# Rouslan/NTracer

Measured on AMD Instinct MI355X. Metric: Mrays/s (primary+shadow), 6-D hypercube @1920x1080, higher is better.
Workload: dtype f32

## Files before the change

### ntracer_amd/csrc/nt_box.hpp

```cpp
#pragma once
#include <type_traits>
#include "nt_pixel.hpp"

namespace {

__device__ __forceinline__ bool box_may_hit(int n, const float *dots, float sx, float sy, float sq) {
    const float osq = dots[0];
    const float ov = fmaf(-dots[2], sy, fmaf(dots[1], sx, dots[3]));
    const float rad2 = (float)n * (1.0f + NT_FUZZ) * (1.0f + NT_FUZZ) * 1.001f;
#ifdef NT_EXP_SKIP_SLABS
    return false;
#else
    return !((osq - rad2) * sq > ov * ov * 1.0001f);
#endif
}

__device__ __forceinline__ void box_background(float in, float &r, float &g, float &b) {
    if (in > 0.0f) { r = in; g = in; b = in; }
    else { r = 0.0f; g = -in; b = -in; }
}

template <int N>
__device__ __forceinline__ void box_color(const float (&o)[N], const float (&dir)[N], bool maybe, float &r, float &g, float &b) {
    bool done = false;
// ... 51 lines not shown

#ifndef NT_BOX_INLINE_MAX_N
#define NT_BOX_INLINE_MAX_N 8
#endif
#ifndef NT_BOX_SETS_MAX_N
#define NT_BOX_SETS_MAX_N NT_BOX_INLINE_MAX_N
#endif
#ifndef NT_BOX_MARGIN
#define NT_BOX_MARGIN 1e-5f
#endif
template <int N>
__device__ __forceinline__ void box_classify(const float (&o)[N], const float (&v)[N], float m, bool maybe, bool &hit, bool &unclear,
                                             float &x, float (&near)[N], float &tn, float &vK) {
    float tn2 = -INFINITY;
    tn = -INFINITY;
    vK = 0.0f;
    float tnp = -INFINITY, tfp = INFINITY;
    const float m1p = 1.0f + m;
#pragma unroll
    for (int j = 0; j < N; ++j) {
        const float inv = __builtin_amdgcn_rcpf(v[j]);
        const float c0 = -o[j] * inv;
        const float nr = c0 - fabsf(inv);
        near[j] = nr;
        tnp = fmaxf(tnp, fmaf(-fabsf(inv), m1p, c0));
        tfp = fminf(tfp, fmaf(fabsf(inv), m1p, c0));
        const bool later = nr > tn;
        tn2 = __builtin_amdgcn_fmed3f(tn, tn2, nr);
        vK = later ? v[j] : vK;
        tn = fmaxf(tn, nr);
    }
    const bool miss = tnp > tfp || tfp < 0.0f;
    const float c = 1.0f - m;
    float sum = 0.0f;
#pragma unroll
    for (int j = 0; j < N; ++j) sum = sum + fmaxf(fabsf(fmaf(v[j], tn, o[j])), c);
    const bool inside = sum - (float)N * c <= 1.5f * m;
    const bool sole = (tn - tn2) * fabsf(vK) > m;
    const bool front = tn > 1e-3f && tn < 1e30f;
    hit = maybe && !miss && inside && sole && front;
    unclear = maybe && !miss && !hit;
#ifdef NT_EXP_NOUNCLEAR
    unclear = false;
#endif
    x = hit ? vK : v[0];
}

__device__ __forceinline__ float nt_vmax(float a, float b) { float r; asm("v_max_f32 %0, %1, %2" : "=v"(r) : "v"(a), "v"(b)); return r; }
__device__ __forceinline__ float nt_vmin(float a, float b) { float r; asm("v_min_f32 %0, %1, %2" : "=v"(r) : "v"(a), "v"(b)); return r; }
__device__ __forceinline__ float nt_vmax3(float a, float b, float c) { float r; asm("v_max3_f32 %0, %1, %2, %3" : "=v"(r) : "v"(a), "v"(b), "v"(c)); return r; }
__device__ __forceinline__ float nt_vmin3(float a, float b, float c) { float r; asm("v_min3_f32 %0, %1, %2, %3" : "=v"(r) : "v"(a), "v"(b), "v"(c)); return r; }
__device__ __forceinline__ float nt_vmed3(float a, float b, float c) { float r; asm("v_med3_f32 %0, %1, %2, %3" : "=v"(r) : "v"(a), "v"(b), "v"(c)); return r; }
__device__ __forceinline__ float nt_vmax_abs(float a, float b) { float r; asm("v_max_f32 %0, |%1|, %2" : "=v"(r) : "v"(a), "v"(b)); return r; }

#ifndef NT_BOX_CLASSIFY_SETS_MIN_N
#define NT_BOX_CLASSIFY_SETS_MIN_N 6
#endif
#ifndef NT_BOX_CLASSIFY_SETS_MAX_N
#define NT_BOX_CLASSIFY_SETS_MAX_N 7
#endif
template <int N>
__device__ __forceinline__ void box_classify_sets(const float (&o)[N], const float (&v)[N], float m, uint32_t sets, bool &hit, bool &unclear,
                                                  float &x) {
    float tn = -INFINITY, tn2 = -INFINITY, vK = 0.0f;
    float tnp = -INFINITY, tfp = INFINITY;
    const float m1p = 1.0f + m;
#pragma unroll
    for (int j = 0; j < N; ++j) {
        if (((sets >> (10 + j)) & 1u) != 0u) {
            const float inv = __builtin_amdgcn_rcpf(v[j]);
            const float c0 = -o[j] * inv;
            tfp = nt_vmin(tfp, fmaf(fabsf(inv), m1p, c0));
            if (((sets >> j) & 1u) != 0u) {
                const float nr = c0 - fabsf(inv);
                tnp = nt_vmax(tnp, fmaf(-fabsf(inv), m1p, c0));
                const bool later = nr > tn;
                tn2 = nt_vmed3(tn, tn2, nr);
                vK = later ? v[j] : vK;
                tn = nt_vmax(tn, nr);
            }
        }
    }
    const bool miss = tnp > tfp || tfp < 0.0f;
    const float c = 1.0f - m;
    float sum = 0.0f;
#ifndef NT_EXP_SETS_MASKS
    asm volatile("" : "+s"(sets));
#endif
#pragma unroll
    for (int j = 0; j < N; ++j) {
        if (((sets >> (10 + j)) & 1u) != 0u) {
            asm volatile("" : "+v"(sum));
            sum = sum + nt_vmax_abs(fmaf(v[j], tn, o[j]), c);
        }
    }
    const bool inside = sum - (float)__builtin_popcount((sets >> 10) & 0x3ffu) * c <= 1.5f * m;
    const bool sole = (tn - tn2) * fabsf(vK) > m;
    const bool front = tn > 1e-3f && tn < 1e30f;
    hit = !miss && inside && sole && front;
    unclear = !miss && !hit;
    x = hit ? vK : v[0];
}

template <int N>
__device__ __forceinline__ void box_entries(const float (&o)[N], const float (&v)[N], float (&near)[N], float &tn, float &vK) {
    tn = -INFINITY;
// ... 56 lines not shown
    }
}

typedef __attribute__((address_space(1))) uint8_t *nt_gptr;
__device__ __forceinline__ nt_gptr uniform_ptr(uint8_t *p) {
    const unsigned long long v = reinterpret_cast<unsigned long long>(p);
    const uint32_t lo = (uint32_t)__builtin_amdgcn_readfirstlane((int)(uint32_t)v), hi = (uint32_t)__builtin_amdgcn_readfirstlane((int)(uint32_t)(v >> 32));
    return (nt_gptr)(((unsigned long long)hi << 32) | lo);
}
#define NT_G32(p) (*(__attribute__((address_space(1))) uint32_t *)(p))

template <typename P>
__device__ __forceinline__ void emit_f32x3_at(const NtTarget &tg, P p, float r, float gb) {
    r = r > 0.0f ? r : 0.0f;
    r = r < 1.0f ? r : 1.0f;
    gb = gb > 0.0f ? gb : 0.0f;
    gb = gb < 1.0f ? gb : 1.0f;
    uint32_t vr = __float_as_uint(r), vgb = __float_as_uint(gb);
    uint3 w;
    if (tg.plain_f32[0] == 0 && tg.plain_f32[1] == 1 && tg.plain_f32[2] == 2 && !tg.reversed) {
        w.x = bswap32(vr);
        w.y = bswap32(vgb);
        w.z = w.y;
    } else {
        if (!tg.reversed) { vr = bswap32(vr); vgb = bswap32(vgb); }
        w.x = tg.plain_f32[tg.reversed ? 2 : 0] == 0 ? vr : vgb;
        w.y = tg.plain_f32[1] == 0 ? vr : vgb;
        w.z = tg.plain_f32[tg.reversed ? 0 : 2] == 0 ? vr : vgb;
    }
    if constexpr (std::is_same<P, nt_gptr>::value) {
        typedef uint32_t u32x3 __attribute__((ext_vector_type(3)));
        u32x3 v;
        v.x = w.x; v.y = w.y; v.z = w.z;
        *(__attribute__((address_space(1))) u32x3 *)(p) = v;
    } else {
        *reinterpret_cast<uint3 *>(p) = w;
    }
}
__device__ __forceinline__ void emit_f32x3(const NtTarget &tg, long long offset, float r, float gb) { emit_f32x3_at(tg, tg.dest + offset, r, gb); }

__device__ __forceinline__ float sqrt_in_range(float x) {
    const float s = __builtin_amdgcn_sqrtf(x);
    const float s_dn = __uint_as_float(__float_as_uint(s) - 1u), s_up = __uint_as_float(__float_as_uint(s) + 1u);
    const float vp = fmaf(-s_dn, s, x), vs = fmaf(-s_up, s, x);
    float r = vp <= 0.0f ? s_dn : s;
    r = vs > 0.0f ? s_up : r;
    return r;
}
__device__ __forceinline__ float sqrt_wave(float x) {
    if (__builtin_amdgcn_ballot_w64(!(x >= 0x1p-96f && x < 0x1p96f)) == 0ull) return sqrt_in_range(x);
    return sqrtf(x);
}

template <int N, bool PLAIN, bool DEFER = false, bool REDO = false, bool F32 = false>
__device__ __forceinline__ bool box_pixel(const NtTarget &tg, const PixelRef &pr, const float (&org)[N], float (&dir)[N], float sq,
                                          const float (&dots)[4], float sx, float sy, float margin, bool rowhit = true, int face = -1,
                                          uint32_t sets = 0u, bool noclass = false) {
    constexpr bool INL = (F32 || PLAIN) && !REDO && !DEFER;
    const bool redo = REDO || (INL && noclass);
    const bool maybe = redo || (rowhit && (DEFER || INL || box_may_hit(N, dots, sx, sy, sq)));
    float r, g, b;
    bool hit = false, unclear = false;
    float x = dir[0];
#ifndef NT_EXP_NOCLASSIFY
    float near[N], tn = 0.0f, vK = 0.0f;
    constexpr bool CSETS = INL && N >= NT_BOX_CLASSIFY_SETS_MIN_N && N <= NT_BOX_CLASSIFY_SETS_MAX_N;
    auto exact_on_sets = [&]() {
        const float len = sqrt_wave(sq);
        float d[N];
#pragma unroll
        for (int j = 0; j < N; ++j) {
            d[j] = 0.0f;
            if ((sets >> (10 + j)) & 1u) d[j] = dir[j] / len;
        }
        bool done = false;
        x = dir[0];
#pragma unroll
        for (int i = 0; i < N; ++i) {
            if (((sets >> i) & 1u) != 0u && __builtin_amdgcn_ballot_w64(!done) != 0ull) {
                const float di = d[i];
                const float dist = ((di < 0.0f ? 1.0f : -1.0f) - org[i]) / di;
                bool ok = !done && di != 0.0f && dist > 0.0f;
#pragma unroll
                for (int j = 0; j < N; ++j) {
                    if (j != i && ((sets >> (10 + j)) & 1u) != 0u) {
                        const float p = d[j] * dist + org[j];
                        ok = ok && !(fabsf(p) > (1.0f + NT_FUZZ));
                    }
                }
                if (ok) {
                    done = true;
                    if (!(dist >= FLT_MAX)) { hit = true; x = dir[i]; }
                }
            }
        }
    };
    if constexpr (CSETS) {
        const bool have_sets = face < 0 && (sets & 0x80000000u) != 0u;
        bool on_sets = have_sets && redo;
        bool sorted = face >= 0;
        if (face >= 0) {
            hit = true;
#pragma unroll
            for (int j = 1; j < N; ++j) x = face == j ? dir[j] : x;
        } else if (have_sets && !redo && __builtin_amdgcn_ballot_w64(maybe) != 0ull) {
            box_classify_sets<N>(org, dir, margin, sets, hit, unclear, x);
            on_sets = __builtin_amdgcn_ballot_w64(unclear) != 0ull;
            unclear = false;
            sorted = true;
        }
        if (on_sets) {
            hit = false;
            exact_on_sets();
        } else if (sorted) {
        } else if (redo) {
            box_entries<N>(org, dir, near, tn, vK);
            unclear = true;
        } else if (__builtin_amdgcn_ballot_w64(maybe) != 0ull) {
            box_classify<N>(org, dir, margin, maybe, hit, unclear, x, near, tn, vK);
        }
    } else {
        if (face >= 0) {
            hit = true;
#pragma unroll
            for (int j = 1; j < N; ++j) x = face == j ? dir[j] : x;
        } else if ((REDO || INL) && redo && (sets & 0x80000000u) != 0u) {
            exact_on_sets();
        } else if (redo) {
            box_entries<N>(org, dir, near, tn, vK);
            unclear = true;
        } else if (__builtin_amdgcn_ballot_w64(maybe) != 0ull) {
            box_classify<N>(org, dir, margin, maybe, hit, unclear, x, near, tn, vK);
        }
    }
    if (DEFER) {
        if (__builtin_amdgcn_ballot_w64(unclear) != 0ull) return false;
    } else {
        const bool hard = unclear && !(tn > 1e-3f && tn < 1e30f);
        if (__builtin_amdgcn_ballot_w64(unclear) != 0ull && __builtin_amdgcn_ballot_w64(hard) == 0ull) {
            box_resolve<N>(org, dir, sqrt_wave(sq), margin, near, tn, vK, unclear, hit, x);
            unclear = false;
        }
    }
#else
    unclear = maybe;
#endif
    if (__builtin_amdgcn_ballot_w64(unclear) == 0ull) {
        if (PLAIN || (plain_rgb(tg) && tg.plain_bits <= 10u)) {
            const float maxv = (float)tg.plain_maxval;
            const float t = (fabsf(x) * __builtin_amdgcn_rsqf(sq)) * maxv;
            const float tgb = hit ? t * 0.5f : t;
            const bool clear_gb = fabsf(__builtin_amdgcn_fractf(tgb) - 0.5f) > fmaf(tgb, 0x1p-20f, 0x1p-20f);
            const bool clear_r = fabsf(__builtin_amdgcn_fractf(t) - 0.5f) > fmaf(t, 0x1p-20f, 0x1p-20f);
            if (__builtin_amdgcn_ballot_w64(!(clear_gb && (clear_r || !hit))) == 0ull) {
                if (tg.plain_sel != 0u) {
                    const uint32_t q8gb = __float_as_uint(tgb + 8388608.0f), q8r = __float_as_uint(t + 8388608.0f);
                    *reinterpret_cast<uint32_t *>(tg.dest + pr.offset) = __builtin_amdgcn_perm((hit || x > 0.0f) ? q8r : 0u, q8gb, tg.plain_sel);
                    return true;
                }
                uint32_t qgb = (uint32_t)(tgb + 0.5f), qr = (uint32_t)(t + 0.5f);
                qgb = qgb < tg.plain_maxval ? qgb : tg.plain_maxval;
                qr = qr < tg.plain_maxval ? qr : tg.plain_maxval;
                emit_plain(tg, pr, (hit || x > 0.0f) ? qr : 0u, qgb);
                return true;
            }
        }
        const float in = x / sqrtf(sq);
        if (hit) {
            const float shade = fabsf(in);
            r = shade * 1.0f;
            g = shade * 0.5f;
            b = shade * 0.5f;
        } else {
            box_background(in, r, g, b);
        }
    } else if (!DEFER) {
        const float len = sqrtf(sq);
#pragma unroll
        for (int j = 0; j < N; ++j) dir[j] = dir[j] / len;
// ... 87 lines not shown
template <int N, int SPLIT>
__global__ __launch_bounds__(256) void box_redo_kernel(NtCameraFixed cam, NtTarget tg) {
    const int tid = (int)threadIdx.x;
    const int wv = __builtin_amdgcn_readfirstlane(tid >> 6);
    static_assert(SPLIT == 1 || SPLIT == 2 || SPLIT == 4, "waves per redo word");
    const int row = (int)blockIdx.y * (4 / SPLIT) + wv / SPLIT;
    if (row >= tg.row_count) return;
    uint32_t *word = tg.redo + ((size_t)blockIdx.z * tg.row_count + row) * tg.redo_words + blockIdx.x;
    const uint32_t mine = (SPLIT == 1 ? 0xffffffffu : SPLIT == 2 ? 0x55555555u : 0x11111111u) << (wv % SPLIT);
    uint32_t todo = *word & mine;
    if (todo == 0u) return;
    if ((tid & 63) == 0) {
        if (SPLIT > 1) atomicAnd(word, ~mine);
        else *word = 0u;
    }
    float org[N], right[N], up[N], fwd[N], dir[N];
    load_camera<N>(cam, org, right, up, fwd);
    float margin = fabsf(org[0]);
#pragma unroll
    for (int j = 1; j < N; ++j) margin = fmaxf(margin, fabsf(org[j]));
    margin = NT_BOX_MARGIN * (1.0f + margin);
    float dots[4];
    if (cam.buf) {
        const float *dp = cam.dots + (size_t)blockIdx.z * 4;
        dots[0] = dp[0]; dots[1] = dp[1]; dots[2] = dp[2]; dots[3] = dp[3];
    } else {
        dots[0] = cam.odots[0]; dots[1] = cam.odots[1]; dots[2] = cam.odots[2]; dots[3] = cam.odots[3];
    }
    const int orow = tg.row_begin + row;
    const int y = nt_image_row(tg, orow);
    if (y >= tg.height) return;
    const float sy = tg.fovI * ((float)y - tg.half_h);
    while (todo != 0u) {
        const int bit = __builtin_ctz(todo);
        todo &= todo - 1u;
        int x = ((int)blockIdx.x * 32 + bit) * 64 + (tid & 63);
        x = x < tg.width ? x : tg.width - 1;
        PixelRef pr;
        pr.x = x;
        pr.y = y;
        pr.offset = (long long)blockIdx.z * tg.frame_stride + (long long)(tg.compact ? orow : y) * tg.pitch + (long long)x * tg.bpp;
        pr.hit_index = 0;
        pr.valid = true;
        const float sx = tg.fovI * ((float)x - tg.half_w);
#pragma unroll
        for (int j = 0; j < N; ++j) dir[j] = (fwd[j] + right[j] * sx) - up[j] * sy;
        float sq = dir[0] * dir[0];
#pragma unroll
        for (int j = 1; j < N; ++j) sq = sq + dir[j] * dir[j];
        box_pixel<N, true, false, true>(tg, pr, org, dir, sq, dots, sx, sy, margin);
    }
}

template <int N, bool SETS = false>
__device__ __forceinline__ unsigned long long box_stretch_code2(const float (&org)[N], const float (&right)[N], const float (&up)[N],
                                                                const float (&fwd)[N], const NtTarget &tg, int y, int col) {
    uint32_t sets_value = 0u;
    uint32_t *const sets = SETS ? &sets_value : nullptr;
    uint32_t code = 0u;
    float omax = fabsf(org[0]);
#pragma unroll
    for (int j = 1; j < N; ++j) omax = fmaxf(omax, fabsf(org[j]));
    const float m = NT_BOX_MARGIN * (1.0f + omax);
    const float h = 1.0f + 2.0f * m + 1e-3f;
    const float sxc = tg.fovI * (((float)(col * 64) + 31.5f) - tg.half_w);
    const float sy = tg.fovI * ((float)y - tg.half_h);
    const float spread = 32.0f * tg.fovI;
    float tlo = 0.0f, thi = INFINITY;
    float vc[N], g[N];
    float tn = -INFINITY, tn2 = -INFINITY, vK = 0.0f, gK = 0.0f, oK = 0.0f;
    int K = 0;
#pragma unroll
    for (int j = 0; j < N; ++j) {
        vc[j] = (fwd[j] + right[j] * sxc) - up[j] * sy;
        g[j] = fmaf(spread, fabsf(right[j]), 1e-6f);
        const float pa = vc[j] + g[j], qa = -h - org[j];
        const float pb = vc[j] - g[j], qb = h - org[j];
        const float ra = qa * __builtin_amdgcn_rcpf(pa), rb = qb * __builtin_amdgcn_rcpf(pb);
        const bool ap = pa >= 0.0f, bp = pb >= 0.0f;
        const float lo_a = ap ? ra : -INFINITY, hi_a = ap ? INFINITY : ra;
        const float hi_b = bp ? rb : INFINITY, lo_b = bp ? -INFINITY : rb;
        tlo = nt_vmax3(tlo, lo_a, lo_b);
        thi = nt_vmin3(thi, hi_a, hi_b);
    }
    if (!(tlo > thi)) {
        code = 15u;
#pragma unroll
        for (int j = 0; j < N; ++j) {
            const float nr = ((vc[j] < 0.0f ? 1.0f : -1.0f) - org[j]) * __builtin_amdgcn_rcpf(vc[j]);
            tn2 = nt_vmed3(tn, tn2, nr);
            const bool later = nr > tn;
            vK = later ? vc[j] : vK;
            gK = later ? g[j] : gK;
            oK = later ? org[j] : oK;
            K = later ? j : K;
            tn = nt_vmax(tn, nr);
        }
        const float vKa = vK - gK, vKb = vK + gK;
        if (K < 13 && vKa * vKb > 0.0f) {
            const float num = (vK < 0.0f ? 1.0f : -1.0f) - oK;
            const float t1 = num * __builtin_amdgcn_rcpf(vKa), t2 = num * __builtin_amdgcn_rcpf(vKb);
            const float t_lo = nt_vmin(t1, t2) * (1.0f - 1e-6f), t_hi = nt_vmax(t1, t2) * (1.0f + 1e-6f);
            const float rK = m * __builtin_amdgcn_rcpf(fabsf(vK) - gK) * (1.0f + 1e-6f);
            bool ok = t_lo > 1e-3f && t_hi < 1e30f;
#pragma unroll
            for (int j = 0; j < N; ++j) {
                const float va = vc[j] - g[j], vb = vc[j] + g[j];
                const float pmax = org[j] + nt_vmax(vb * t_lo, vb * t_hi);
                const float pmin = org[j] + nt_vmin(va * t_lo, va * t_hi);
                const float lim = (1.0f - m - 1e-4f) - (fabsf(vc[j]) + g[j]) * rK;
                ok = ok && (j == K || (pmax <= lim && pmin >= -lim));
            }
            if (ok) code = (uint32_t)K + 1u;
        }
        if (code == 15u && !((tn - tn2) * fabsf(vK) > m)) code = 14u;
        if (code >= 14u) {
            if (sets != nullptr && N <= 10) {
                auto range = [&](int j, float &A, float &B, float &vabs) {
                    const float va = vc[j] - g[j], vb = vc[j] + g[j];
                    const float num = (vc[j] < 0.0f ? 1.0f : -1.0f) - org[j];
                    const float e1 = num * __builtin_amdgcn_rcpf(va), e2 = num * __builtin_amdgcn_rcpf(vb);
                    const float lo = nt_vmin(e1, e2), hi = nt_vmax(e1, e2);
                    const bool same = va * vb > 0.0f;
                    A = same ? lo - fabsf(lo) * 1e-6f : -INFINITY;
                    B = same ? hi + fabsf(hi) * 1e-6f : INFINITY;
                    vabs = same ? fabsf(vc[j]) - g[j] : 0.0f;
                };
                float rA[N], rB[N], rV[N];
                float TN = -INFINITY, TH = -INFINITY;
#pragma unroll
                for (int j = 0; j < N; ++j) {
                    range(j, rA[j], rB[j], rV[j]);
                    TN = nt_vmax(TN, rA[j]);
                    TH = nt_vmax(TH, rB[j]);
                }
                float vmin = INFINITY;
#pragma unroll
                for (int j = 0; j < N; ++j) vmin = rB[j] >= TN ? nt_vmin(vmin, rV[j]) : vmin;
                const float M = m * __builtin_amdgcn_rcpf(vmin) * (1.0f + 1e-5f);
                uint32_t T = 0u, C = 0u;
                float t_lo = INFINITY;
                const float t_hi = TH;
#pragma unroll
                for (int j = 0; j < N; ++j) {
                    const bool inT = rB[j] >= TN - M;
                    T |= inT ? 1u << j : 0u;
                    t_lo = inT ? nt_vmin(t_lo, rA[j]) : t_lo;
                }
#pragma unroll
                for (int j = 0; j < N; ++j) {
                    const float va = vc[j] - g[j], vb = vc[j] + g[j];
                    const float pmax = org[j] + nt_vmax(vb * t_lo, vb * t_hi);
                    const float pmin = org[j] + nt_vmin(va * t_lo, va * t_hi);
                    const float lim = 1.0f - m - 1e-4f;
                    const bool inC = ((T >> j) & 1u) != 0u || !(pmax <= lim && pmin >= -lim);
                    C |= inC ? 1u << j : 0u;
                }
                const bool valid = vmin > 0.0f && t_lo > 1e-3f && t_hi < 1e30f;
                *sets = valid ? (0x80000000u | (C << 10) | T) : 0u;
            }
        }
    }
    return (unsigned long long)code | ((unsigned long long)sets_value << 32);
}
template <int N>
__device__ __forceinline__ uint32_t box_stretch_code(const float (&org)[N], const float (&right)[N], const float (&up)[N], const float (&fwd)[N],
                                                     const NtTarget &tg, int y, int col) {
    return (uint32_t)box_stretch_code2<N, false>(org, right, up, fwd, tg, y, col);
}

template <int N>
__global__ __launch_bounds__(256) void box_cull_kernel(NtCameraFixed cam, NtTarget tg, uint32_t *out, int ncols) {
    float org[N], right[N], up[N], fwd[N];
    load_camera<N>(cam, org, right, up, fwd);
    const int word = (int)blockIdx.x, row = (int)blockIdx.y * 8 + (int)(threadIdx.x >> 5);
    const int col = word * 32 + (int)(threadIdx.x & 31);
    uint32_t code = 0u;
    if (row < tg.row_count && col < ncols) {
        const int orow = tg.row_begin + row;
        const int y = nt_image_row(tg, orow);
        code = box_stretch_code<N>(org, right, up, fwd, tg, y, col);
    }
    uint32_t packed = code << (4 * (threadIdx.x & 7));
    packed |= (uint32_t)__shfl_xor((int)packed, 1, 64);
    packed |= (uint32_t)__shfl_xor((int)packed, 2, 64);
    packed |= (uint32_t)__shfl_xor((int)packed, 4, 64);
    if (row < tg.row_count && (threadIdx.x & 7) == 0) out[((size_t)blockIdx.z * tg.row_count + row) * tg.cull_words + (col >> 3)] = packed;
}

#ifdef NT_EXP_NOSTORE
#define NT_EXP_STORE_IF if (tg.width < 0)
#else
#define NT_EXP_STORE_IF
#endif
#ifndef NT_TILE_OCC
#define NT_TILE_OCC
#endif
#ifndef NT_BOX_PIN_UP
#define NT_BOX_PIN_UP 1
#endif
#ifndef NT_BOX_LEAN_GROUPS_MAX_N
#define NT_BOX_LEAN_GROUPS_MAX_N 20
#endif
__device__ __forceinline__ bool guard_clear(float t) { return fabsf(__builtin_amdgcn_fractf(t) - 0.5f) > fmaf(t, 0x1p-18f, 0x1p-18f); }
__device__ __forceinline__ float lean_quotient(float d, float sy, float uu, float m2bu, float bb) {
    return fabsf(d) * __builtin_amdgcn_rsqf(fmaf(sy, fmaf(sy, uu, m2bu), bb));
}
template <int N>
__device__ __forceinline__ void pick_component(uint32_t K, const float (&base)[N], const float (&upv)[N], float &bK, float &uK) {
    bK = base[0];
    uK = upv[0];
#pragma unroll
    for (int j = 1; j < N; ++j) {
        bK = K == (uint32_t)j ? base[j] : bK;
        uK = K == (uint32_t)j ? upv[j] : uK;
    }
}
template <int N>
__device__ __forceinline__ float row_dir(const float (&base)[N], const float (&upv)[N], float sy, float (&dir)[N]) {
#pragma unroll
    for (int j = 0; j < N; ++j) dir[j] = base[j] - upv[j] * sy;
    float sq = dir[0] * dir[0];
#pragma unroll
    for (int j = 1; j < N; ++j) sq = sq + dir[j] * dir[j];
    return sq;
}
#ifndef NT_BOX_PASS_ROWS
#define NT_BOX_PASS_ROWS 64
#endif
__device__ __forceinline__ int nt_low_bit(uint32_t m) { return __builtin_ctz(m); }
__device__ __forceinline__ int nt_low_bit(unsigned long long m) { return __builtin_ctzll(m); }
__device__ __forceinline__ int nt_count_bits(uint32_t m) { return __builtin_popcount(m); }
__device__ __forceinline__ int nt_count_bits(unsigned long long m) { return __builtin_popcountll(m); }
__device__ __forceinline__ void nt_clear_bit(uint32_t &m, int bit) { asm("s_bitset0_b32 %0, %1" : "+s"(m) : "s"(bit)); }
__device__ __forceinline__ void nt_clear_bit(unsigned long long &m, int bit) { asm("s_bitset0_b64 %0, %1" : "+s"(m) : "s"(bit)); }
__device__ __forceinline__ void nt_set_bit(uint32_t &m, int bit) { asm("s_bitset1_b32 %0, %1" : "+s"(m) : "s"(bit)); }
__device__ __forceinline__ void nt_set_bit(unsigned long long &m, int bit) { asm("s_bitset1_b64 %0, %1" : "+s"(m) : "s"(bit)); }
__device__ __forceinline__ void nt_drop_low_bit(uint32_t &m, int) { m &= m - 1u; }
__device__ __forceinline__ void nt_drop_low_bit(unsigned long long &m, int bit) { nt_clear_bit(m, bit); }
template <int N, bool F32, int ROWS, int WAVES>
__global__ __launch_bounds__(64 * WAVES) NT_TILE_OCC void box_tile_kernel(NtCameraFixed cam, NtTarget tg) {
    static_assert(ROWS == 8 || ROWS == 16 || ROWS == 64, "a wave's rows: a qword of sixteen codes in LDS or fewer, or one row a lane");
    static_assert(WAVES >= 1 && WAVES <= 4 && WAVES * ROWS <= 64, "the codes of a tile are the work of one wave, a row per lane");
    static_assert(WAVES == 1 ? ROWS == 64 : ROWS <= 16, "one wave a block renders the 64 rows whose codes it worked out itself");
    constexpr int R = ROWS;
    constexpr bool REG = WAVES == 1;
    constexpr int LDS_N = REG ? 1 : 64;
    __shared__ uint32_t s_code[LDS_N];
    __shared__ unsigned long long s_rows[REG ? 1 : 4];
    constexpr bool ALLIN = F32 || N <= NT_BOX_INLINE_MAX_N;
    constexpr bool SETS_LDS = ALLIN && N <= NT_BOX_SETS_MAX_N;
    __shared__ uint32_t s_sets[SETS_LDS ? LDS_N : 1];
    __shared__ int s_abort;
    uint32_t lane_cs = 0u;
    const int tid = (int)threadIdx.x;
    const int lane = tid & 63;
    const int wv = __builtin_amdgcn_readfirstlane(tid >> 6);
#ifdef NT_EXP_TRACE
    const unsigned long long trace_t0 = wall_clock64();
    unsigned trace_rows = 0u;
    unsigned long long trace_t1 = 0ull;
#endif
    const unsigned nframes = gridDim.z - (unsigned)tg.lead_frames;
    unsigned frame = blockIdx.z;
    if (tg.lead_frames > 0) {
        const unsigned cols = gridDim.x, q = cols / 4u;
        const bool middle = blockIdx.x >= q && blockIdx.x < cols - q;
        if (!middle) frame -= (unsigned)tg.lead_frames;
        if (frame >= nframes) return;
    }
    float org[N], right[N], up[N], fwd[N], dir[N];
    load_camera<N>(cam, frame, org, right, up, fwd);
    float margin = fabsf(org[0]);
#pragma unroll
    for (int j = 1; j < N; ++j) margin = fmaxf(margin, fabsf(org[j]));
    margin = NT_BOX_MARGIN * (1.0f + margin);
    float dots[4];
    if (cam.buf) {
        const float *dp = cam.dots + (size_t)frame * 4;
        dots[0] = dp[0]; dots[1] = dp[1]; dots[2] = dp[2]; dots[3] = dp[3];
    } else {
        dots[0] = cam.odots[0]; dots[1] = cam.odots[1]; dots[2] = cam.odots[2]; dots[3] = cam.odots[3];
    }
    const int tile_row0 = (int)blockIdx.y * WAVES * R;
    if (REG || wv == (int)((blockIdx.x + blockIdx.y + frame) % (unsigned)WAVES)) {
        if (tg.abort_word != nullptr) {
            const bool ab = nt_aborted(tg);
            if constexpr (REG) { if (ab) return; }
            else { if (lane == 0) s_abort = ab ? 1 : 0; }
        }
        uint32_t code = 0u;
        uint32_t row_sets = 0u;
        const int trow = tg.row_il > 0 ? ((int)blockIdx.y * WAVES + lane / R) + tg.row_il * (lane % R) : tile_row0 + lane;
        if (lane < WAVES * R && trow < tg.row_count) {
            const int orow = tg.row_begin + trow;
            const int y = nt_image_row(tg, orow);
            if (y < tg.height) {
                const unsigned long long cs = box_stretch_code2<N, (N <= NT_BOX_SETS_MAX_N)>(org, right, up, fwd, tg, y, (int)blockIdx.x);
                code = (uint32_t)cs;
                row_sets = (uint32_t)(cs >> 32);
            }
        }
        if constexpr (REG) {
            lane_cs = (SETS_LDS ? row_sets & 0x800fffffu : 0u) | (code << 20);
        } else {
            if (SETS_LDS) s_sets[lane] = row_sets;
            {
                const unsigned long long m0 = __builtin_amdgcn_ballot_w64(code == 0u), m1 = __builtin_amdgcn_ballot_w64(code >= 1u && code <= 13u),
                                         m2 = __builtin_amdgcn_ballot_w64(code == 15u), m3 = __builtin_amdgcn_ballot_w64(code == 14u);
                if (lane == 0) {
                    s_rows[0] = m0;
                    s_rows[1] = m1;
                    s_rows[2] = m2;
                    s_rows[3] = m3;
                }
            }
            uint32_t packed = code << (4 * (lane & 7));
            packed |= (uint32_t)__shfl_xor((int)packed, 1, 64);
            packed |= (uint32_t)__shfl_xor((int)packed, 2, 64);
            packed |= (uint32_t)__shfl_xor((int)packed, 4, 64);
            if ((lane & 7) == 0) {
                const int grp = lane >> 3;
                const int slot = R == 8 ? 2 * grp : grp;
                s_code[slot] = packed;
                if (R == 8) s_code[slot + 1] = 0u;
            }
        }
    }
    if constexpr (!REG) {
        __syncthreads();
        if (tg.abort_word != nullptr && s_abort != 0) return;
    }
#ifdef NT_EXP_TRACE
    trace_t1 = wall_clock64();
#endif
    constexpr int PASS = R == 64 ? NT_BOX_PASS_ROWS : R;
    static_assert(PASS == R || (R == 64 && PASS == 16), "NT_BOX_PASS_ROWS: 64 or 16");
    typedef typename std::conditional<PASS == 64, unsigned long long, uint32_t>::type mask_t;
    const int wrow0 = tile_row0 + wv * R;
    const int il = tg.row_il;
    const int wfirst = il > 0 ? (int)blockIdx.y * WAVES + wv : wrow0;
    if (wfirst < tg.row_count) {
        typedef uint32_t nt_u32x4 __attribute__((ext_vector_type(4)));
        typedef __attribute__((address_space(4))) const nt_u32x4 *nt_rowtab;
        typedef uint32_t nt_u32x16 __attribute__((ext_vector_type(16), aligned(16)));
        typedef __attribute__((address_space(4))) const nt_u32x16 *nt_rowtab4;
        constexpr bool GROUPS = !F32 && N <= NT_BOX_LEAN_GROUPS_MAX_N;
        uint8_t *const frame_base = tg.dest + (long long)frame * tg.frame_stride;
#define NT_ROW_LOAD(rr)                     \
        const nt_u32x4 row_e = tab[(rr)];   \
        const float sy = __uint_as_float(row_e.x)
#define NT_ROW_OFF() ((long long)(((unsigned long long)row_e.w << 32) | row_e.z) + (long long)frame * tg.frame_stride)
#define NT_ROW_PTR() uniform_ptr(frame_base + (long long)(((unsigned long long)row_e.w << 32) | row_e.z))
#define NT_GROUP_PTR(k) uniform_ptr(frame_base + (long long)(((unsigned long long)grp_e[4 * (k) + 3] << 32) | grp_e[4 * (k) + 2]))
#define NT_LANE_OFF() ({ asm volatile("" : "+v"(xoff)); xoff; })
#define NT_CLEAR_BIT(mask, bit) nt_clear_bit(mask, bit)
#define NT_SET_BIT(mask, bit) nt_set_bit(mask, bit)
// ... 16 lines not shown
#pragma unroll
            for (int j = 0; j < N; ++j) {
                bb = fmaf(base[j], base[j], bb);
                bu = fmaf(base[j], up[j], bu);
                uu = fmaf(up[j], up[j], uu);
            }
            fastsq = __builtin_amdgcn_ballot_w64(!(bu * bu <= bb * uu * 0.0625f)) == 0ull;
        }
        const float maxv = (float)tg.plain_maxval;
        const float inv_maxv2 = 1.0f / (maxv * maxv);
        const float m2bu = (-2.0f * bu) * inv_maxv2;
        bb = bb * inv_maxv2;
        uu = uu * inv_maxv2;
        const uint32_t lane_code = (lane_cs >> 20) & 15u;
        unsigned long long rows_culled, rows_face, rows_rays, rows_tie;
        if constexpr (REG) {
            rows_culled = __builtin_amdgcn_ballot_w64(lane_code == 0u);
            rows_face = __builtin_amdgcn_ballot_w64(lane_code >= 1u && lane_code <= 13u);
            rows_rays = __builtin_amdgcn_ballot_w64(lane_code == 15u);
            rows_tie = __builtin_amdgcn_ballot_w64(lane_code == 14u);
        } else {
            auto rows_of = [&](int k) {
                const unsigned long long m = s_rows[k];
                return (((unsigned long long)(uint32_t)__builtin_amdgcn_readfirstlane((int)(uint32_t)(m >> 32)) << 32) |
                        (uint32_t)__builtin_amdgcn_readfirstlane((int)(uint32_t)m)) >> (wv * R);
            };
            rows_culled = rows_of(0);
            rows_face = rows_of(1);
            rows_rays = rows_of(2);
            rows_tie = rows_of(3);
        }
        const int lrow = il > 0 ? wfirst + il * lane : wrow0 + lane;
        const int ly = nt_image_row(tg, tg.row_begin + lrow);
        const unsigned long long rows_valid = __builtin_amdgcn_ballot_w64(lane < R && lrow < tg.row_count && ly < tg.height);
#pragma unroll 1
        for (int pass = 0; pass < R / PASS; ++pass) {
        const int slot0 = PASS * pass;
        const int row0 = wrow0 + slot0;
        const int hfirst = il > 0 ? wfirst + il * slot0 : row0;
        if (hfirst >= tg.row_count) break;
        mask_t redo_bits = 0u;
        unsigned long long rowcodes = 0ull;
        if constexpr (!REG) {
            rowcodes = ((unsigned long long)(uint32_t)__builtin_amdgcn_readfirstlane((int)s_code[2 * wv + 1]) << 32) |
                       (uint32_t)__builtin_amdgcn_readfirstlane((int)s_code[2 * wv]);
        }
        auto slot_word = [&](int rr) { return (uint32_t)__builtin_amdgcn_readlane((int)lane_cs, slot0 + rr); };
        auto code_of = [&](int rr) {
            if constexpr (REG) return (slot_word(rr) >> 20) & 15u;
            else return (uint32_t)(rowcodes >> (4 * rr)) & 15u;
        };
        auto sets_of = [&](int rr) {
            if constexpr (!SETS_LDS) return 0u;
            else if constexpr (REG) return slot_word(rr) & 0x800fffffu;
            else return (uint32_t)__builtin_amdgcn_readfirstlane((int)s_sets[wv * R + rr]);
        };
        auto rows_with_code = [&](uint32_t c) {
            if constexpr (REG) return (mask_t)(__builtin_amdgcn_ballot_w64(lane_code == c) >> slot0);
            else return (mask_t)__builtin_amdgcn_ballot_w64(lane < PASS && ((uint32_t)(rowcodes >> (4 * (lane & 15))) & 15u) == c);
        };
        const mask_t valid = R > PASS ? (mask_t)(rows_valid >> slot0) & (mask_t)((1ull << (PASS & 63)) - 1ull) : (mask_t)rows_valid;
        const nt_rowtab tab = (nt_rowtab)tg.rowtab + (il > 0 ? row0 : tg.row_begin + row0);
        mask_t quick = (mask_t)(rows_culled >> slot0) & valid, inner = (mask_t)(rows_face >> slot0) & valid;
        mask_t todo = (mask_t)((ALLIN ? rows_rays | rows_tie : rows_rays) >> slot0) & valid;
        if (!ALLIN) redo_bits = (mask_t)(rows_tie >> slot0) & valid;
#ifdef NT_EXP_TRACE
        trace_rows += (unsigned)nt_count_bits(quick) | ((unsigned)nt_count_bits(inner) << 8) |
                      ((unsigned)nt_count_bits((mask_t)(rows_rays >> slot0) & valid) << 16) |
                      ((unsigned)nt_count_bits((mask_t)(rows_tie >> slot0) & valid) << 24);
#endif
        if (!F32) {
            if (!fastsq) {
                todo |= quick | inner;
                quick = 0u;
                inner = 0u;
            }
            auto lean_rows = [&](auto sel8) {
            constexpr bool SEL8 = decltype(sel8)::value;
#ifdef NT_EXP_RED_BY_SHIFT
#define NT_RED_OF(q, d0) ((q) & (uint32_t)((int32_t)__float_as_uint(d0) >> 31))
#else
#define NT_RED_OF(q, d0) ((d0) > 0.0f ? (q) : 0u)
#endif
            auto put_quick = [&](nt_gptr out, float t, float d0) {
                if (SEL8) {
                    const uint32_t q = __float_as_uint(t + 8388608.0f);
                    NT_EXP_STORE_IF NT_G32(out) = __builtin_amdgcn_perm(NT_RED_OF(q, d0), q, tg.plain_sel);
                    return;
                }
                uint32_t q = (uint32_t)(t + 0.5f);
                q = q < tg.plain_maxval ? q : tg.plain_maxval;
                const uint32_t w = NT_RED_OF(q, d0) * tg.plain_mul[0] + q * (tg.plain_mul[1] + tg.plain_mul[2]);
                NT_EXP_STORE_IF NT_G32(out) = tg.reversed ? w : bswap32(w);
            };
            auto put_face = [&](nt_gptr out, float t, float th) {
                if (SEL8) {
                    NT_EXP_STORE_IF NT_G32(out) = __builtin_amdgcn_perm(__float_as_uint(t + 8388608.0f), __float_as_uint(th + 8388608.0f), tg.plain_sel);
                    return;
                }
                uint32_t qr = (uint32_t)(t + 0.5f), qgb = (uint32_t)(th + 0.5f);
                qr = qr < tg.plain_maxval ? qr : tg.plain_maxval;
                qgb = qgb < tg.plain_maxval ? qgb : tg.plain_maxval;
                const uint32_t w = qr * tg.plain_mul[0] + qgb * (tg.plain_mul[1] + tg.plain_mul[2]);
                NT_EXP_STORE_IF NT_G32(out) = tg.reversed ? w : bswap32(w);
            };
            auto full_groups = [](mask_t mask) { return mask & (mask >> 1) & (mask >> 2) & (mask >> 3) & (mask_t)(PASS == 64 ? 0x1111111111111111ull : 0x1111ull); };
            auto lean_group = [&](int g, auto row, auto put) {
// ... 79 lines not shown
                    float t, th;
                    if (__builtin_expect(__builtin_amdgcn_ballot_w64(!face_row(bK0, uK0, sy, t, th)) == 0ull, 1)) {
                        put_face(NT_ROW_PTR() + NT_LANE_OFF(), t, th);
                        NT_SET_BIT(same_stored, rr);
                    }
                }
                todo |= same & ~same_stored;
            }
            };
            if (tg.plain_sel != 0u) lean_rows(std::true_type{});
            else lean_rows(std::false_type{});
        } else {
            while (quick != 0u) {
                const int rr = nt_low_bit(quick);
                nt_drop_low_bit(quick, rr);
                NT_ROW_LOAD(rr);
                const float sq = row_dir<N>(base, upv, sy, dir);
                const float in = dir[0] / sqrt_wave(sq);
                float r, gb, b_;
                box_background(in, r, gb, b_);
                emit_f32x3_at(tg, NT_ROW_PTR() + NT_LANE_OFF(), r, gb);
            }
            while (inner != 0u) {
                const uint32_t code0 = code_of(nt_low_bit(inner));
                float bK0, uK0;
                pick_component<N>(code0 - 1u, base, upv, bK0, uK0);
                mask_t same = inner & rows_with_code(code0);
                inner &= ~same;
                while (same != 0u) {
                    const int rr = nt_low_bit(same);
                    nt_drop_low_bit(same, rr);
                    NT_ROW_LOAD(rr);
                    const float sq = row_dir<N>(base, upv, sy, dir);
                    const float xk = bK0 - uK0 * sy;
                    const float shade = fabsf(xk / sqrt_wave(sq));
                    emit_f32x3_at(tg, NT_ROW_PTR() + NT_LANE_OFF(), shade * 1.0f, shade * 0.5f);
                }
            }
        }
        while (todo != 0u) {
            const int rr = nt_low_bit(todo);
            nt_drop_low_bit(todo, rr);
            const int rcode = (int)code_of(rr);
            const bool rowhit = rcode != 0;
            NT_ROW_LOAD(rr);
            PixelRef pr;
            pr.x = x;
            pr.y = 0;
            pr.offset = NT_ROW_OFF() + (long long)xoff;
            pr.hit_index = 0;
            pr.valid = true;
            const float sq = row_dir<N>(base, upv, sy, dir);
            if (ALLIN) {
                box_pixel<N, !F32, false, false, F32>(tg, pr, org, dir, sq, dots, sx, sy, margin, rowhit, rcode >= 1 && rcode <= 13 ? rcode - 1 : -1,
                                                       sets_of(rr), rcode == 14);
            } else if (!box_pixel<N, true, true, false, false>(tg, pr, org, dir, sq, dots, sx, sy, margin, rowhit, rcode >= 1 && rcode <= 13 ? rcode - 1 : -1)) {
                redo_bits |= (mask_t)1u << rr;
            }
        }
        if (!ALLIN && lane == 0) {
            while (redo_bits != 0u) {
                const int rr = nt_low_bit(redo_bits);
                nt_drop_low_bit(redo_bits, rr);
                const int mrow = il > 0 ? hfirst + il * rr : row0 + rr;
                atomicOr(tg.redo + ((size_t)frame * tg.row_count + mrow) * tg.redo_words + (blockIdx.x >> 5), 1u << (blockIdx.x & 31));
            }
        }
        }
    }
#ifdef NT_EXP_TRACE
    if (lane == 0) {
        unsigned long long *tr = reinterpret_cast<unsigned long long *>(tg.dest + (long long)nframes * tg.frame_stride) +
                                 ((((size_t)frame * gridDim.y + blockIdx.y) * gridDim.x + blockIdx.x) * WAVES + wv) * 4;
        tr[0] = trace_t0;
        tr[1] = wall_clock64();
        tr[2] = (unsigned long long)__builtin_amdgcn_s_getreg(4 | (31 << 11)) | ((unsigned long long)__builtin_amdgcn_s_getreg(20 | (31 << 11)) << 32);
        tr[3] = (unsigned long long)trace_rows | ((trace_t1 - trace_t0) << 32);
    }
#endif
#undef NT_ROW_LOAD
#undef NT_ROW_OFF
#undef NT_ROW_PTR
#undef NT_GROUP_PTR
#undef NT_LANE_OFF
#undef NT_CLEAR_BIT
#undef NT_SET_BIT
#undef NT_RED_OF
}

template <int N>
int launch_box_fixed(const NtLaunchInfo &li, const NtCamera &cam, const NtTarget &tg_in) {
    NtCameraFixed cf;
    cf.buf = cam.buf;
    cf.dots = cam.dots;
    for (int k = 0; k < 4; ++k) cf.odots[k] = cam.odots[k];
    cf.n = N;
    for (int k = 0; k < 4 * N; ++k) cf.inl[k] = cam.inl[k];
    NtTarget tg = tg_in;
    dim3 grid;
    grid_for(tg, 64, tg.colors_out ? 4 : 4 * NT_BOXROWS, li.nframes, grid);
    tg.cull = nullptr;
    tg.redo = nullptr;
    tg.cull_words = 0;
    tg.redo_words = 0;
    const bool fmt_rgb = tg.plain_bits != 0u && tg.plain_bits <= 10u && tg.bpp == 4 && tg.aligned4;
    const bool fmt_f32 = tg.plain_f32[0] >= 0 && tg.bpp == 12 && tg.aligned4;
    if (li.cull_buf && tg.rowtab && !tg.colors_out && (fmt_rgb || fmt_f32) && li.cull_clean) {
        hipStream_t st = (hipStream_t)li.stream;
        NtBoxTileGeom geom;
        geom.rows = li.tile_rows;
        geom.waves = li.tile_waves;
        const bool r64 = geom.rows == 64, r16 = geom.rows == 16;
        const int wpb = geom.waves;
        const int tile_rows = geom.rows * geom.waves;
        dim3 tgrid((unsigned)((tg.width + 63) / 64), (unsigned)((tg.row_count + tile_rows - 1) / tile_rows), (unsigned)li.nframes);
        tg.redo_words = ((tg.width + 63) / 64 + 31) / 32;
        tg.redo = li.cull_buf;
        tg.lead_frames = li.nframes >= 8 ? (li.nframes < 96 ? li.nframes : 96) : 0;
        if (tg.row_il > 0) tg.lead_frames = li.nframes >= 32 ? 16 : 0;
        if ((long long)li.nframes + tg.lead_frames > 65535) tg.lead_frames = 0;
        tgrid.z += (unsigned)tg.lead_frames;
        if (fmt_rgb) {
            if (r64) hipLaunchKernelGGL((box_tile_kernel<N, false, 64, 1>), tgrid, dim3(64), 0, st, cf, tg);
            else if (r16 && wpb == 3) hipLaunchKernelGGL((box_tile_kernel<N, false, 16, 3>), tgrid, dim3(192), 0, st, cf, tg);
            else if (r16) hipLaunchKernelGGL((box_tile_kernel<N, false, 16, 4>), tgrid, dim3(256), 0, st, cf, tg);
            else hipLaunchKernelGGL((box_tile_kernel<N, false, 8, 4>), tgrid, dim3(256), 0, st, cf, tg);
            if constexpr (N > NT_BOX_INLINE_MAX_N) {
                const long long rwords = (long long)tg.row_count * li.nframes * tg.redo_words;
                const int split = rwords < 48 * 1024 ? 2 : 1;
                const int rpb = 4 / split;
                const dim3 rgrid((unsigned)tg.redo_words, (unsigned)((tg.row_count + rpb - 1) / rpb), (unsigned)li.nframes);
                if (split == 2) hipLaunchKernelGGL((box_redo_kernel<N, 2>), rgrid, dim3(256), 0, st, cf, tg);
                else hipLaunchKernelGGL((box_redo_kernel<N, 1>), rgrid, dim3(256), 0, st, cf, tg);
            }
        } else {
            if (r64) hipLaunchKernelGGL((box_tile_kernel<N, true, 64, 1>), tgrid, dim3(64), 0, st, cf, tg);
            else if (r16 && wpb == 3) hipLaunchKernelGGL((box_tile_kernel<N, true, 16, 3>), tgrid, dim3(192), 0, st, cf, tg);
            else if (r16) hipLaunchKernelGGL((box_tile_kernel<N, true, 16, 4>), tgrid, dim3(256), 0, st, cf, tg);
            else hipLaunchKernelGGL((box_tile_kernel<N, true, 8, 4>), tgrid, dim3(256), 0, st, cf, tg);
        }
        return 0;
    }
    if (li.cull_buf && !tg.colors_out) {
        const int ncols = (tg.width + 63) / 64;
        const int words = (ncols + 31) / 32;
        tg.cull_words = 4 * words;
        hipLaunchKernelGGL(box_cull_kernel<N>, dim3((unsigned)words, (unsigned)((tg.row_count + 7) / 8), (unsigned)li.nframes), dim3(256), 0,
                           (hipStream_t)li.stream, cf, tg, li.cull_buf, ncols);
        tg.cull = li.cull_buf;
    }
    hipLaunchKernelGGL(box_kernel<N>, grid, dim3(256), 0, (hipStream_t)li.stream, cf, tg);
    return 0;
}

}
```

### ntracer_amd/csrc/nt_inst_box.hip

```cpp
#ifndef NT_INST_N
#error "one dimension a translation unit: compile with -DNT_INST_N=<N> (build.py)"
#endif
#if !defined(NT_TILE_OCC)
#if NT_INST_N <= 5
#define NT_TILE_OCC __attribute__((amdgpu_num_sgpr(96)))
#elif NT_INST_N == 6
#define NT_TILE_OCC __attribute__((amdgpu_waves_per_eu(7, 7), amdgpu_num_sgpr(96)))
#define NT_BOX_PIN_UP 0
#elif NT_INST_N == 10
#define NT_TILE_OCC __attribute__((amdgpu_waves_per_eu(5, 5)))
#elif NT_INST_N == 15
#define NT_TILE_OCC __attribute__((amdgpu_waves_per_eu(4, 4)))
#elif NT_INST_N >= 21 && NT_INST_N <= 24
#define NT_TILE_OCC __attribute__((amdgpu_waves_per_eu(3, 3)))
#endif
#endif
#include "nt_box.hpp"
#include "nt_dispatch.hpp"

template <> int nt_box_fixed<NT_INST_N>(const NtLaunchInfo &li, const NtCamera &cam, const NtTarget &tg) {
    return launch_box_fixed<NT_INST_N>(li, cam, tg);
}
```

Before: 1.072 million.

## Add sure-hit shortcut that writes quantized color without exact set tests

During row classification, a new flag marks rows where the hit face set equals the candidate set, the origin is near the box, and the direction spread across the tile is small. For pixels on such rows, the kernel bounds the quantized color from the min and max hit-axis direction components. When the whole wave agrees the rounding is unambiguous, it writes the packed RGB directly and skips the exact per-axis intersection loop. This adds extra code-classification work and register pressure, and it is enabled only for the 64-row tile layout with large grids in dimensions 6 and 8.

```diff
diff --git a/ntracer_amd/csrc/nt_box.hpp b/ntracer_amd/csrc/nt_box.hpp
--- a/ntracer_amd/csrc/nt_box.hpp
+++ b/ntracer_amd/csrc/nt_box.hpp
@@ -127,6 +127,27 @@
 __device__ __forceinline__ float nt_vmin3(float a, float b, float c) { float r; asm("v_min3_f32 %0, %1, %2, %3" : "=v"(r) : "v"(a), "v"(b), "v"(c)); return r; }
 __device__ __forceinline__ float nt_vmed3(float a, float b, float c) { float r; asm("v_med3_f32 %0, %1, %2, %3" : "=v"(r) : "v"(a), "v"(b), "v"(c)); return r; }
 __device__ __forceinline__ float nt_vmax_abs(float a, float b) { float r; asm("v_max_f32 %0, |%1|, %2" : "=v"(r) : "v"(a), "v"(b)); return r; }
+__device__ __forceinline__ float nt_vmax3_abs(float a, float b, float c) { float r; asm("v_max3_f32 %0, %1, |%2|, |%3|" : "=v"(r) : "v"(a), "v"(b), "v"(c)); return r; }
+__device__ __forceinline__ float nt_vmin_abs(float a, float b) { float r; asm("v_min_f32 %0, |%1|, %2" : "=v"(r) : "v"(a), "v"(b)); return r; }
+
+#ifndef NT_BOX_TIE_SHORTCUT
+#define NT_BOX_TIE_SHORTCUT 1
+#endif
+#ifndef NT_BOX_TIE_SHORTCUT_MIN_N
+#define NT_BOX_TIE_SHORTCUT_MIN_N 6
+#endif
+#ifndef NT_BOX_TIE_SHORTCUT_MAX_N
+#define NT_BOX_TIE_SHORTCUT_MAX_N 8
+#endif
+#ifndef NT_BOX_TIE_SURE_MAX_ORIGIN
+#define NT_BOX_TIE_SURE_MAX_ORIGIN 4.5f
+#endif
+#ifndef NT_BOX_TIE_SHORTCUT_MIN_WAVES
+#define NT_BOX_TIE_SHORTCUT_MIN_WAVES 32768
+#endif
+#define NT_BOX_SETS_SURE 0x01000000u
+template <int N>
+constexpr bool nt_box_tie_shortcut() { return NT_BOX_TIE_SHORTCUT != 0 && N >= NT_BOX_TIE_SHORTCUT_MIN_N && N <= NT_BOX_TIE_SHORTCUT_MAX_N && N <= NT_BOX_SETS_MAX_N; }
 
 #ifndef NT_BOX_CLASSIFY_SETS_MIN_N
 #define NT_BOX_CLASSIFY_SETS_MIN_N 6
@@ -289,7 +310,7 @@
     return sqrtf(x);
 }
 
-template <int N, bool PLAIN, bool DEFER = false, bool REDO = false, bool F32 = false>
+template <int N, bool PLAIN, bool DEFER = false, bool REDO = false, bool F32 = false, bool TIE = false>
 __device__ __forceinline__ bool box_pixel(const NtTarget &tg, const PixelRef &pr, const float (&org)[N], float (&dir)[N], float sq,
                                           const float (&dots)[4], float sx, float sy, float margin, bool rowhit = true, int face = -1,
                                           uint32_t sets = 0u, bool noclass = false) {
@@ -332,6 +353,36 @@
             }
         }
     };
+    constexpr bool SURE = TIE && nt_box_tie_shortcut<N>() && INL && PLAIN && !F32;
+    auto sure_hit_row = [&]() -> bool {
+        float lo = INFINITY, hi = 0.0f;
+#pragma unroll
+        for (int j = 0; j < N; ++j) {
+            if (((sets >> j) & 1u) != 0u) {
+                asm volatile("" : "+v"(lo), "+v"(hi));
+                lo = nt_vmin_abs(dir[j], lo);
+                hi = nt_vmax_abs(dir[j], hi);
+            }
+        }
+        const float maxv = (float)tg.plain_maxval;
+        const float rs = __builtin_amdgcn_rsqf(sq);
+        const float t0 = (lo * rs) * maxv, t1 = (hi * rs) * maxv;
+        const float h0 = t0 * 0.5f, h1 = t1 * 0.5f;
+        auto clear = [](float t) { return fabsf(__builtin_amdgcn_fractf(t) - 0.5f) > fmaf(t, 0x1p-20f, 0x1p-20f); };
+        const uint32_t r0 = __float_as_uint(t0 + 8388608.0f), r1 = __float_as_uint(t1 + 8388608.0f);
+        const uint32_t g0 = __float_as_uint(h0 + 8388608.0f), g1 = __float_as_uint(h1 + 8388608.0f);
+        const bool same = clear(t0) && clear(t1) && clear(h0) && clear(h1) && r0 == r1 && g0 == g1;
+        if (__builtin_amdgcn_ballot_w64(!same) != 0ull) return false;
+        if (tg.plain_sel != 0u) {
+            *reinterpret_cast<uint32_t *>(tg.dest + pr.offset) = __builtin_amdgcn_perm(r1, g1, tg.plain_sel);
+            return true;
+        }
+        uint32_t qgb = (uint32_t)(h1 + 0.5f), qr = (uint32_t)(t1 + 0.5f);
+        qgb = qgb < tg.plain_maxval ? qgb : tg.plain_maxval;
+        qr = qr < tg.plain_maxval ? qr : tg.plain_maxval;
+        emit_plain(tg, pr, qr, qgb);
+        return true;
+    };
     if constexpr (CSETS) {
         const bool have_sets = face < 0 && (sets & 0x80000000u) != 0u;
         bool on_sets = have_sets && redo;
@@ -347,6 +398,9 @@
             sorted = true;
         }
         if (on_sets) {
+            if constexpr (SURE) {
+                if ((sets & NT_BOX_SETS_SURE) != 0u && redo && sure_hit_row()) return true;
+            }
             hit = false;
             exact_on_sets();
         } else if (sorted) {
@@ -362,6 +416,9 @@
 #pragma unroll
             for (int j = 1; j < N; ++j) x = face == j ? dir[j] : x;
         } else if ((REDO || INL) && redo && (sets & 0x80000000u) != 0u) {
+            if constexpr (SURE) {
+                if ((sets & NT_BOX_SETS_SURE) != 0u && sure_hit_row()) return true;
+            }
             exact_on_sets();
         } else if (redo) {
             box_entries<N>(org, dir, near, tn, vK);
@@ -555,7 +612,7 @@
     }
 }
 
-template <int N, bool SETS = false>
+template <int N, bool SETS = false, bool SURE = false>
 __device__ __forceinline__ unsigned long long box_stretch_code2(const float (&org)[N], const float (&right)[N], const float (&up)[N],
                                                                 const float (&fwd)[N], const NtTarget &tg, int y, int col) {
     uint32_t sets_value = 0u;
@@ -661,6 +718,17 @@
                 }
                 const bool valid = vmin > 0.0f && t_lo > 1e-3f && t_hi < 1e30f;
                 *sets = valid ? (0x80000000u | (C << 10) | T) : 0u;
+                if constexpr (SURE) {
+                    float wmax = 0.0f;
+                    uint32_t far_axes = 0u;
+#pragma unroll
+                    for (int j = 0; j < N; ++j) {
+                        wmax = nt_vmax3_abs(wmax, vc[j] - g[j], vc[j] + g[j]);
+                        far_axes |= (__float_as_uint(org[j]) & 0x7fffffffu) > __float_as_uint(NT_BOX_TIE_SURE_MAX_ORIGIN) ? 1u << j : 0u;
+                    }
+                    const bool sure = valid && C == T && (T & far_axes) == 0u && (t_hi - t_lo) * wmax <= 1.0f;
+                    *sets |= sure ? NT_BOX_SETS_SURE : 0u;
+                }
             }
         }
     }
@@ -741,8 +809,9 @@
 __device__ __forceinline__ void nt_set_bit(unsigned long long &m, int bit) { asm("s_bitset1_b64 %0, %1" : "+s"(m) : "s"(bit)); }
 __device__ __forceinline__ void nt_drop_low_bit(uint32_t &m, int) { m &= m - 1u; }
 __device__ __forceinline__ void nt_drop_low_bit(unsigned long long &m, int bit) { nt_clear_bit(m, bit); }
-template <int N, bool F32, int ROWS, int WAVES>
+template <int N, bool F32, int ROWS, int WAVES, bool TIE = false>
 __global__ __launch_bounds__(64 * WAVES) NT_TILE_OCC void box_tile_kernel(NtCameraFixed cam, NtTarget tg) {
+    static_assert(!TIE || (!F32 && ROWS == 64 && nt_box_tie_shortcut<N>()), "the short cut: packed RGB, 64 x 1, the dimensions it is built for");
     static_assert(ROWS == 8 || ROWS == 16 || ROWS == 64, "a wave's rows: a qword of sixteen codes in LDS or fewer, or one row a lane");
     static_assert(WAVES >= 1 && WAVES <= 4 && WAVES * ROWS <= 64, "the codes of a tile are the work of one wave, a row per lane");
     static_assert(WAVES == 1 ? ROWS == 64 : ROWS <= 16, "one wave a block renders the 64 rows whose codes it worked out itself");
@@ -753,6 +822,7 @@
     __shared__ unsigned long long s_rows[REG ? 1 : 4];
     constexpr bool ALLIN = F32 || N <= NT_BOX_INLINE_MAX_N;
     constexpr bool SETS_LDS = ALLIN && N <= NT_BOX_SETS_MAX_N;
+    constexpr uint32_t SETS_MASK = 0x800fffffu | (TIE ? NT_BOX_SETS_SURE : 0u);
     __shared__ uint32_t s_sets[SETS_LDS ? LDS_N : 1];
     __shared__ int s_abort;
     uint32_t lane_cs = 0u;
@@ -799,13 +869,13 @@
             const int orow = tg.row_begin + trow;
             const int y = nt_image_row(tg, orow);
             if (y < tg.height) {
-                const unsigned long long cs = box_stretch_code2<N, (N <= NT_BOX_SETS_MAX_N)>(org, right, up, fwd, tg, y, (int)blockIdx.x);
+                const unsigned long long cs = box_stretch_code2<N, (N <= NT_BOX_SETS_MAX_N), TIE>(org, right, up, fwd, tg, y, (int)blockIdx.x);
                 code = (uint32_t)cs;
                 row_sets = (uint32_t)(cs >> 32);
             }
         }
         if constexpr (REG) {
-            lane_cs = (SETS_LDS ? row_sets & 0x800fffffu : 0u) | (code << 20);
+            lane_cs = (SETS_LDS ? row_sets & SETS_MASK : 0u) | (code << 20);
         } else {
             if (SETS_LDS) s_sets[lane] = row_sets;
             {
@@ -928,7 +998,7 @@
         };
         auto sets_of = [&](int rr) {
             if constexpr (!SETS_LDS) return 0u;
-            else if constexpr (REG) return slot_word(rr) & 0x800fffffu;
+            else if constexpr (REG) return slot_word(rr) & SETS_MASK;
             else return (uint32_t)__builtin_amdgcn_readfirstlane((int)s_sets[wv * R + rr]);
         };
         auto rows_with_code = [&](uint32_t c) {
@@ -1114,7 +1184,7 @@
             pr.valid = true;
             const float sq = row_dir<N>(base, upv, sy, dir);
             if (ALLIN) {
-                box_pixel<N, !F32, false, false, F32>(tg, pr, org, dir, sq, dots, sx, sy, margin, rowhit, rcode >= 1 && rcode <= 13 ? rcode - 1 : -1,
+                box_pixel<N, !F32, false, false, F32, TIE>(tg, pr, org, dir, sq, dots, sx, sy, margin, rowhit, rcode >= 1 && rcode <= 13 ? rcode - 1 : -1,
                                                        sets_of(rr), rcode == 14);
             } else if (!box_pixel<N, true, true, false, false>(tg, pr, org, dir, sq, dots, sx, sy, margin, rowhit, rcode >= 1 && rcode <= 13 ? rcode - 1 : -1)) {
                 redo_bits |= (mask_t)1u << rr;
@@ -1183,7 +1253,11 @@
         if ((long long)li.nframes + tg.lead_frames > 65535) tg.lead_frames = 0;
         tgrid.z += (unsigned)tg.lead_frames;
         if (fmt_rgb) {
-            if (r64) hipLaunchKernelGGL((box_tile_kernel<N, false, 64, 1>), tgrid, dim3(64), 0, st, cf, tg);
+            bool tie = false;
+            if constexpr (nt_box_tie_shortcut<N>()) tie = r64 && (unsigned long long)tgrid.x * tgrid.y * (unsigned)li.nframes >= (unsigned long long)NT_BOX_TIE_SHORTCUT_MIN_WAVES;
+            if (tie) {
+                if constexpr (nt_box_tie_shortcut<N>()) hipLaunchKernelGGL((box_tile_kernel<N, false, 64, 1, true>), tgrid, dim3(64), 0, st, cf, tg);
+            } else if (r64) hipLaunchKernelGGL((box_tile_kernel<N, false, 64, 1>), tgrid, dim3(64), 0, st, cf, tg);
             else if (r16 && wpb == 3) hipLaunchKernelGGL((box_tile_kernel<N, false, 16, 3>), tgrid, dim3(192), 0, st, cf, tg);
             else if (r16) hipLaunchKernelGGL((box_tile_kernel<N, false, 16, 4>), tgrid, dim3(256), 0, st, cf, tg);
             else hipLaunchKernelGGL((box_tile_kernel<N, false, 8, 4>), tgrid, dim3(256), 0, st, cf, tg);
diff --git a/ntracer_amd/csrc/nt_inst_box.hip b/ntracer_amd/csrc/nt_inst_box.hip
--- a/ntracer_amd/csrc/nt_inst_box.hip
+++ b/ntracer_amd/csrc/nt_inst_box.hip
@@ -15,6 +15,9 @@
 #define NT_TILE_OCC __attribute__((amdgpu_waves_per_eu(3, 3)))
 #endif
 #endif
+#if NT_INST_N == 7 && !defined(NT_BOX_TIE_SHORTCUT)
+#define NT_BOX_TIE_SHORTCUT 0
+#endif
 #include "nt_box.hpp"
 #include "nt_dispatch.hpp"
 
```

Result: faster. 1.087 million (median of 6 runs) (+1.4%).
